# dps/rust-raytracer

Measured on NVIDIA H100. Metric: Mrays/sec (primary+scattered), higher is better.
Workload: dtype f64

## Files before the change

rust-raytracer_b200/csrc/rtb200_trace.cuh:

```cuda
#pragma once
#include "rtb200_kernels.cuh"

namespace rtk {

using namespace rtd;

#ifndef RT_SCATTER_TRIPS
#define RT_SCATTER_TRIPS 2
#endif
#ifndef RT_SMEM_STACK
#define RT_SMEM_STACK 10
#endif

enum : uint32_t { CLS_MISS = 0, CLS_DIFFUSE = 1, CLS_METAL = 2, CLS_GLASS = 3, CLS_LIGHT = 4, CLS_DEAD = 5, N_CLS = 6 };
constexpr uint32_t kDeadLevel = 0xffffffffu;
constexpr uint32_t kScatterPending = 0x80000000u;
using rtbvh::kLeafBit;
constexpr unsigned long long kNoHitBits = 0x7ff0000000000000ull;
constexpr uint32_t kNoSphere = 0xffffffffu;
using rtbvh::kSkipNodeBit;
using rtbvh::kNoSkip;
constexpr uint32_t kSlotBytes = 7 * 8 + 10 * 4 + RT_SMEM_STACK * 4;
constexpr uint32_t kFrameSlotBytes = 4;

struct Pool {
    double *ox, *oy, *oz, *dx, *dy, *dz, *bt;
    uint32_t *bi, *work, *pix, *smp, *blk, *clo, *chi, *lvl, *shd;
    uint32_t *src;
    uint32_t *stk;
    uint32_t *frm;
    uint32_t n_slots;
    uint32_t stack_col;
};
RT_DEV Pool pool_at(unsigned char* base, uint32_t n_slots, uint32_t stack_col) {
    Pool P;
    double* d = reinterpret_cast<double*>(base);
    P.ox = d; P.oy = d + n_slots; P.oz = d + 2 * n_slots; P.dx = d + 3 * n_slots; P.dy = d + 4 * n_slots; P.dz = d + 5 * n_slots; P.bt = d + 6 * n_slots;
    uint32_t* u = reinterpret_cast<uint32_t*>(d + 7 * n_slots);
    P.bi = u; P.work = u + n_slots; P.pix = u + 2 * n_slots; P.smp = u + 3 * n_slots; P.blk = u + 4 * n_slots; P.clo = u + 5 * n_slots;
    P.chi = u + 6 * n_slots; P.lvl = u + 7 * n_slots; P.shd = u + 8 * n_slots; P.src = u + 9 * n_slots; P.stk = u + 10 * n_slots;
    P.frm = u + (10 + RT_SMEM_STACK) * n_slots;
    P.n_slots = n_slots; P.stack_col = stack_col;
    return P;
}

struct WarpCtx {
    float4 *cA, *cB, *cC;
    uint32_t *skip;
    uint32_t *l_in, *l_lf, *l_cd;
};
constexpr uint32_t kWarpCtxBytes = (3 * 32 * 16 + 32 * 4 + (uint32_t)(kCapIn + kCapLf + kCapCd) * 4 + 15u) & ~15u;
RT_DEV WarpCtx warpctx_at(unsigned char* base) {
    WarpCtx W;
    W.cA = reinterpret_cast<float4*>(base); W.cB = W.cA + 32; W.cC = W.cB + 32;
    W.skip = reinterpret_cast<uint32_t*>(W.cC + 32);
    W.l_in = W.skip + 32; W.l_lf = W.l_in + kCapIn; W.l_cd = W.l_lf + kCapLf;
    return W;
}

struct SceneRefs {
    const float4* nodes; const float4* leaf_rec; const uint32_t* leaf_id; const float4* filt;
    const double4* geo; const DevMat* mat;
};

struct Stats {
    uint32_t rays = 0, cand = 0, ovf = 0, samples = 0, leaves = 0, nodes = 0;
#if RT_PHASE_CLOCKS
    unsigned long long t_node = 0, t_leaf = 0, t_exact = 0;
    uint32_t exact_steps = 0, exact_tests = 0, src_skips = 0;
#endif
};

RT_DEV void bulk_stage(void* dst, const void* src, uint32_t bytes, uint64_t* bar) {
    const uint32_t CH = 32768u;
    for (uint32_t o = 0; o < bytes; o += CH) {
        uint32_t nb = bytes - o < CH ? bytes - o : CH;
        tma_bulk_g2s((char*)dst + o, (const char*)src + o, nb, bar);
    }
}

RT_DEV void albedo_of(uint32_t code, const DevMat* mat, float& r, float& g, float& b) {
    if (code == 0xffffffffu) { r = g = b = 1.0f; return; }
    if (code & 0x80000000u) {
        r = __fdiv_rn((float)(code & 0xffu), 255.0f);
        g = __fdiv_rn((float)((code >> 8) & 0xffu), 255.0f);
        b = __fdiv_rn((float)((code >> 16) & 0xffu), 255.0f);
    } else {
        const DevMat& m = mat[code];
        r = m.r; g = m.g; b = m.b;
    }
}

RT_DEV float fmax3(float a, float b, float c) { return fmaxf(fmaxf(a, b), c); }
RT_DEV float fmin3(float a, float b, float c) { return fminf(fminf(a, b), c); }

RT_DEV uint32_t warp_scan_incl(uint32_t v, int lane) {
#pragma unroll
    for (int off = 1; off < 32; off <<= 1) {
        uint32_t t = __shfl_up_sync(0xffffffffu, v, off);
        if (lane >= off) v += t;
    }
    return v;
}

RT_DEV float2 fma2_rn(float2 a, float2 b, float2 c) { return make_float2(__fmaf_rn(a.x, b.x, c.x), __fmaf_rn(a.y, b.y, c.y)); }

#define RT_FILTER_PAIRS(REC, DV, NP)                                                                                                  \
    _Pragma("unroll") for (int q = 0; q < (NP); ++q) {                                                                              \
        float4 A_ = (REC)[2 * q], B_ = (REC)[2 * q + 1];                                                                             \
        float2 cx = make_float2(A_.x, A_.y), cy = make_float2(A_.z, A_.w), cz = make_float2(B_.x, B_.y), nk = make_float2(B_.z, B_.w); \
        float2 bb = fma2_rn(cz, dz2, nod2);                                                                                          \
        float2 tt = fma2_rn(cz, oz2, nk);                                                                                            \
        bb = fma2_rn(cy, dy2, bb);                                                                                                   \
        tt = fma2_rn(cy, oy2, tt);                                                                                                   \
        bb = fma2_rn(cx, dx2, bb);                                                                                                   \
        tt = fma2_rn(cx, ox2, tt);                                                                                                   \
        (DV)[q] = fma2_rn(bb, bb, tt);                                                                                               \
    }

RT_DEV uint32_t class_of(uint32_t kind) {
    return (kind == RT_METAL) ? CLS_METAL : (kind == RT_GLASS) ? CLS_GLASS : (kind == RT_LIGHT) ? CLS_LIGHT : CLS_DIFFUSE;
}

template <uint32_t MODE, bool ANY = false>
RT_DEV uint32_t closest_hit(const TraceParams& p, const SceneRefs& sc, const Pool& P, const WarpCtx& W, bool alive, uint32_t slot, int lane, Stats& st,
                            double t_hi = DBL_MAX, float* tcap = nullptr) {
    const unsigned FULL = 0xffffffffu;
    uint32_t cls = CLS_DEAD;
    if (__ballot_sync(FULL, alive) == 0u) return cls;
    const uint32_t lt_mask = (1u << lane) - 1u;
    unsigned long long* btu = reinterpret_cast<unsigned long long*>(P.bt);
    const D3 o = mk(P.ox[slot], P.oy[slot], P.oz[slot]), d = mk(P.dx[slot], P.dy[slot], P.dz[slot]);
    const double a = length_squared(d);
    const double thi = ANY ? t_hi : DBL_MAX;
    bool ovf = false;
    uint32_t done = 0u;
    double best_t = DBL_MAX;
    int best = -1;
    auto confirm = [&](int j) {
        if constexpr (ANY) { if (best >= 0) return; }
        double4 gq = sc.geo[j];
        double root;
        if (sphere_root(mk(gq.x, gq.y, gq.z), gq.w, o, d, a, 0.001, thi, root)) {
            if (best < 0 || root < best_t || (root == best_t && j < best)) { best_t = root; best = j; }
        }
        ++st.cand;
    };
    if (alive) { btu[slot] = kNoHitBits; P.bi[slot] = 0xffffffffu; }
    if (MODE != MODE_EXACT) {
        const float ofx = __double2float_rn(__dsub_rn(o.x, p.gx)), ofy = __double2float_rn(__dsub_rn(o.y, p.gy)),
                    ofz = __double2float_rn(__dsub_rn(o.z, p.gz));
        const float dfx = __double2float_rn(d.x), dfy = __double2float_rn(d.y), dfz = __double2float_rn(d.z);
        const float s = fmaf(dfx, dfx, fmaf(dfy, dfy, dfz * dfz));
        const float oo = fmaf(ofx, ofx, fmaf(ofy, ofy, ofz * ofz));
        const bool ok = (s > 1e-30f) && (s < 1e30f) && (oo < 1e30f);
        const float inv = rsqrtf(s);
        const float dnx = dfx * inv, dny = dfy * inv, dnz = dfz * inv;
        const float nod = -fmaf(ofx, dnx, fmaf(ofy, dny, ofz * dnz));
        const float thr = __fmul_rd(oo, p.er_coef);
        if (alive && !ok) ovf = true;
        if (MODE == MODE_TREE) {
            const float ax = fabsf(dnx) < 1e-20f ? copysignf(1e-20f, dnx) : dnx;
            const float ay = fabsf(dny) < 1e-20f ? copysignf(1e-20f, dny) : dny;
            const float az = fabsf(dnz) < 1e-20f ? copysignf(1e-20f, dnz) : dnz;
            const float mray = __fmul_ru(1.9073486328125e-6f, __fsqrt_ru(oo));
            W.cA[lane] = make_float4(ofx, ofy, ofz, mray);
            W.cB[lane] = make_float4(__frcp_rn(ax), __frcp_rn(ay), __frcp_rn(az), thr);
            W.cC[lane] = make_float4(dnx, dny, dnz, nod);
            if constexpr (ANY) tcap[lane] = __double2float_ru(__dmul_ru(__dmul_ru(t_hi, __dsqrt_ru(a)), 1.0 + 0x1p-40));
            uint32_t skp = kNoSkip;
            const uint32_t src = alive ? P.src[slot] : kNoSphere;
            if (src != kNoSphere) {
                const uint32_t pos = p.skip_pos[src];
                const double4 gs = sc.geo[src];
                if (pos != kNoSkip && leaves_sphere(mk(gs.x, gs.y, gs.z), gs.w, o, d, a)) skp = pos;
            }
            W.skip[lane] = skp;
            const uint32_t fat_in = (uint32_t)kCapIn - 7u * p.depth - 8u;
            const bool enter = alive && ok && p.n_nodes != 0u;
            const unsigned em = __ballot_sync(FULL, enter);
            uint32_t n_in = (uint32_t)__popc(em), n_lf = 0u, n_cd = 0u;
            if (enter) W.l_in[__popc(em & lt_mask)] = (uint32_t)lane;
            __syncwarp();
            uint32_t guard = 0;
            for (;;) {
#if RT_PHASE_CLOCKS
                const unsigned long long t_step = clock64();
#endif
                if (n_in != 0u && n_lf <= (uint32_t)(kCapLf - 64)) {
                    const uint32_t m = n_in < 32u ? n_in : 32u;
                    const bool act = (uint32_t)lane < m;
                    const uint32_t e = act ? W.l_in[n_in - 1u - (uint32_t)lane] : 0u;
                    const uint32_t ray = e & 31u, node = e >> 5;
                    uint32_t hit = 0u, leafbits = 0u;
                    const float4* N = sc.nodes + (size_t)node * kNodeVec;
                    bool test = act;
                    if constexpr (ANY) test = act && !((done >> ray) & 1u);
                    if (test) {
                        const float4 A = W.cA[ray], B = W.cB[ray];
                        float tcr = 0.f;
                        if constexpr (ANY) tcr = tcap[ray];
                        auto far_ = [&](float f) { if constexpr (ANY) return fminf(f, tcr); else return f; };
                        const uint32_t sx = __float_as_uint(B.x) >> 31, sy = __float_as_uint(B.y) >> 31, sz = __float_as_uint(B.z) >> 31;
                        const float mx = copysignf(A.w, B.x), my = copysignf(A.w, B.y), mz = copysignf(A.w, B.z);
                        const float cnx = __fmul_rn(__fadd_rn(A.x, mx), -B.x), cfx = __fmul_rn(__fsub_rn(A.x, mx), -B.x);
                        const float cny = __fmul_rn(__fadd_rn(A.y, my), -B.y), cfy = __fmul_rn(__fsub_rn(A.y, my), -B.y);
                        const float cnz = __fmul_rn(__fadd_rn(A.z, mz), -B.z), cfz = __fmul_rn(__fsub_rn(A.z, mz), -B.z);
                        const float2 ix2 = make_float2(B.x, B.x), iy2 = make_float2(B.y, B.y), iz2 = make_float2(B.z, B.z);
                        const float2 cnx2 = make_float2(cnx, cnx), cny2 = make_float2(cny, cny), cnz2 = make_float2(cnz, cnz);
                        const float2 cfx2 = make_float2(cfx, cfx), cfy2 = make_float2(cfy, cfy), cfz2 = make_float2(cfz, cfz);
                        const float4* Nnx = N + (sx ? 6 : 0); const float4* Nfx = N + (sx ? 0 : 6);
                        const float4* Nny = N + (sy ? 8 : 2); const float4* Nfy = N + (sy ? 2 : 8);
                        const float4* Nnz = N + (sz ? 10 : 4); const float4* Nfz = N + (sz ? 4 : 10);
#pragma unroll
                        for (int h = 0; h < 2; ++h) {
                            const float4 NX = Nnx[h], NY = Nny[h], NZ = Nnz[h], FX = Nfx[h], FY = Nfy[h], FZ = Nfz[h];
                            const float2 tnx0 = fma2_rn(make_float2(NX.x, NX.y), ix2, cnx2), tnx1 = fma2_rn(make_float2(NX.z, NX.w), ix2, cnx2);
                            const float2 tny0 = fma2_rn(make_float2(NY.x, NY.y), iy2, cny2), tny1 = fma2_rn(make_float2(NY.z, NY.w), iy2, cny2);
                            const float2 tnz0 = fma2_rn(make_float2(NZ.x, NZ.y), iz2, cnz2), tnz1 = fma2_rn(make_float2(NZ.z, NZ.w), iz2, cnz2);
                            const float2 tfx0 = fma2_rn(make_float2(FX.x, FX.y), ix2, cfx2), tfx1 = fma2_rn(make_float2(FX.z, FX.w), ix2, cfx2);
                            const float2 tfy0 = fma2_rn(make_float2(FY.x, FY.y), iy2, cfy2), tfy1 = fma2_rn(make_float2(FY.z, FY.w), iy2, cfy2);
                            const float2 tfz0 = fma2_rn(make_float2(FZ.x, FZ.y), iz2, cfz2), tfz1 = fma2_rn(make_float2(FZ.z, FZ.w), iz2, cfz2);
                            hit |= (fmaxf(fmax3(tnx0.x, tny0.x, tnz0.x), 0.f) <= far_(fmin3(tfx0.x, tfy0.x, tfz0.x)) ? 1u : 0u) << (4 * h + 0);
                            hit |= (fmaxf(fmax3(tnx0.y, tny0.y, tnz0.y), 0.f) <= far_(fmin3(tfx0.y, tfy0.y, tfz0.y)) ? 1u : 0u) << (4 * h + 1);
                            hit |= (fmaxf(fmax3(tnx1.x, tny1.x, tnz1.x), 0.f) <= far_(fmin3(tfx1.x, tfy1.x, tfz1.x)) ? 1u : 0u) << (4 * h + 2);
                            hit |= (fmaxf(fmax3(tnx1.y, tny1.y, tnz1.y), 0.f) <= far_(fmin3(tfx1.y, tfy1.y, tfz1.y)) ? 1u : 0u) << (4 * h + 3);
                        }
                        const uint4 R0 = *reinterpret_cast<const uint4*>(N + kChildVec), R1 = *reinterpret_cast<const uint4*>(N + kChildVec + 1);
                        leafbits = (R0.x >> 31) | ((R0.y >> 31) << 1) | ((R0.z >> 31) << 2) | ((R0.w >> 31) << 3) |
                                   ((R1.x >> 31) << 4) | ((R1.y >> 31) << 5) | ((R1.z >> 31) << 6) | ((R1.w >> 31) << 7);
                    }
                    {
                        const uint32_t sk = W.skip[ray] ^ (kSkipNodeBit | node << 3);
                        if (sk < 8u) {
#if RT_PHASE_CLOCKS
                            st.src_skips += (hit >> sk) & 1u;
#endif
                            hit &= ~(1u << sk);
                        }
                    }
                    const uint32_t packed = (uint32_t)__popc(hit & ~leafbits) | ((uint32_t)__popc(hit & leafbits) << 16);
                    const uint32_t inc = warp_scan_incl(packed, lane);
                    const uint32_t new_in = n_in - ((uint32_t)lane + 1u) + (inc & 0xffffu);
                    const bool fits = new_in <= (lane == 0 ? (uint32_t)kCapIn : fat_in) && n_lf + (inc >> 16) <= (uint32_t)kCapLf;
                    const unsigned okm = __ballot_sync(FULL, fits || !act);
                    uint32_t k = okm == FULL ? 32u : (uint32_t)(__ffs(~okm) - 1);
                    k = k < m ? k : m;
                    if (k == 0u) { if (lane == 0) atomicAdd(&p.err[1], 1ull); break; }
                    const uint32_t tot = __shfl_sync(FULL, inc, (int)k - 1);
                    __syncwarp();
                    if (act && (uint32_t)lane < k) {
                        const uint32_t exc = inc - packed;
                        uint32_t pi = (n_in - k) + (exc & 0xffffu), pl = n_lf + (exc >> 16);
                        const uint32_t* refs = reinterpret_cast<const uint32_t*>(N + kChildVec);
                        uint32_t mm = hit;
                        while (mm) {
                            const int c = __ffs(mm) - 1;
                            mm &= mm - 1u;
                            const uint32_t ref = refs[c];
                            if (ref & kLeafBit) W.l_lf[pl++] = (ref << 5) | ray;
                            else W.l_in[pi++] = (ref << 5) | ray;
                        }
                        if constexpr (ANY) st.nodes += test ? 1u : 0u; else ++st.nodes;
                    }
                    n_in = n_in - k + (tot & 0xffffu);
                    n_lf += tot >> 16;
                    __syncwarp();
#if RT_PHASE_CLOCKS
                    if (lane == 0) st.t_node += clock64() - t_step;
#endif
                } else if (n_lf != 0u && n_cd <= (uint32_t)(kCapCd - 32)) {
                    const uint32_t m = n_lf < 32u ? n_lf : 32u;
                    const bool act = (uint32_t)lane < m;
                    const uint32_t e = act ? W.l_lf[n_lf - 1u - (uint32_t)lane] : 0u;
                    const uint32_t ray = e & 31u, leaf = e >> 5;
                    uint32_t hit = 0u;
                    bool test = act;
                    if constexpr (ANY) test = act && !((done >> ray) & 1u);
                    if (test) {
                        const float4 A = W.cA[ray], C = W.cC[ray];
                        const float th = W.cB[ray].w;
                        const float2 dx2 = make_float2(C.x, C.x), dy2 = make_float2(C.y, C.y), dz2 = make_float2(C.z, C.z);
                        const float2 ox2 = make_float2(2.f * A.x, 2.f * A.x), oy2 = make_float2(2.f * A.y, 2.f * A.y), oz2 = make_float2(2.f * A.z, 2.f * A.z);
                        const float2 nod2 = make_float2(C.w, C.w);
                        float2 Dv[kLeafK / 2];
                        const float4* rec = sc.leaf_rec + (size_t)leaf * kLeafK;
                        RT_FILTER_PAIRS(rec, Dv, kLeafK / 2)
#pragma unroll
                        for (int q = 0; q < kLeafK / 2; ++q) hit |= (Dv[q].x >= th ? 1u : 0u) << (2 * q) | (Dv[q].y >= th ? 1u : 0u) << (2 * q + 1);
                        const uint32_t sk = W.skip[ray];
                        if (sk / (uint32_t)kLeafK == leaf) {
#if RT_PHASE_CLOCKS
                            st.src_skips += (hit >> (sk % (uint32_t)kLeafK)) & 1u;
#endif
                            hit &= ~(1u << (sk % (uint32_t)kLeafK));
                        }
                    }
                    const uint32_t cntc = (uint32_t)__popc(hit);
                    const uint32_t inc = warp_scan_incl(cntc, lane);
                    const bool fits = n_cd + inc <= (uint32_t)kCapCd;
                    const unsigned okm = __ballot_sync(FULL, fits || !act);
                    uint32_t k = okm == FULL ? 32u : (uint32_t)(__ffs(~okm) - 1);
                    k = k < m ? k : m;
                    if (k == 0u) { if (lane == 0) atomicAdd(&p.err[1], 1ull); break; }
                    const uint32_t tot = __shfl_sync(FULL, inc, (int)k - 1);
                    if (act && (uint32_t)lane < k) {
                        uint32_t pc = n_cd + inc - cntc;
                        const uint32_t* ids = sc.leaf_id + (size_t)leaf * kLeafK;
                        uint32_t mm = hit;
                        while (mm) {
                            const int c = __ffs(mm) - 1;
                            mm &= mm - 1u;
                            W.l_cd[pc++] = (ids[c] << 5) | ray;
                        }
                        if constexpr (ANY) st.leaves += test ? 1u : 0u; else ++st.leaves;
                    }
                    n_lf -= k;
                    n_cd += tot;
                    __syncwarp();
#if RT_PHASE_CLOCKS
                    if (lane == 0) st.t_leaf += clock64() - t_step;
#endif
                } else if (n_cd != 0u) {
                    const uint32_t m = n_cd < 32u ? n_cd : 32u;
                    const bool act = (uint32_t)lane < m;
                    const uint32_t e = act ? W.l_cd[n_cd - 1u - (uint32_t)lane] : 0u;
                    const uint32_t rs = __shfl_sync(FULL, slot, (int)(e & 31u)), sph = e >> 5;
                    if constexpr (ANY) {
                        const uint32_t ray = e & 31u;
                        const double tr = __shfl_sync(FULL, t_hi, (int)ray);
                        bool acc = false;
                        if (act && !((done >> ray) & 1u)) {
                            const D3 ro = mk(P.ox[rs], P.oy[rs], P.oz[rs]), rd = mk(P.dx[rs], P.dy[rs], P.dz[rs]);
                            const double4 gq = sc.geo[sph];
                            double root;
                            acc = sphere_root(mk(gq.x, gq.y, gq.z), gq.w, ro, rd, length_squared(rd), 0.001, tr, root);
                            ++st.cand;
#if RT_PHASE_CLOCKS
                            ++st.exact_tests;
#endif
                        }
                        if (acc) P.bi[rs] = sph;
                        done |= __reduce_or_sync(FULL, acc ? 1u << ray : 0u);
                        n_cd -= m;
                        __syncwarp();
                        if ((em & ~done) == 0u) break;
                    } else {
                        unsigned long long key = ~0ull;
                        if (act) {
                            const D3 ro = mk(P.ox[rs], P.oy[rs], P.oz[rs]), rd = mk(P.dx[rs], P.dy[rs], P.dz[rs]);
                            const double4 gq = sc.geo[sph];
                            double root;
                            if (sphere_root(mk(gq.x, gq.y, gq.z), gq.w, ro, rd, length_squared(rd), 0.001, DBL_MAX, root)) key = (unsigned long long)__double_as_longlong(root);
                            ++st.cand;
#if RT_PHASE_CLOCKS
                            ++st.exact_tests;
#endif
                        }
                        const bool h = key != ~0ull;
                        const unsigned long long before = h ? btu[rs] : 0ull;
                        __syncwarp();
                        if (h && key < before) atomicMin(&btu[rs], key);
                        __syncwarp();
                        const bool mine = h && key == btu[rs];
                        if (mine && key < before) atomicMax(&P.bi[rs], 0xffffffffu);
                        __syncwarp();
                        if (mine) atomicMin(&P.bi[rs], sph);
                        n_cd -= m;
                        __syncwarp();
                    }
#if RT_PHASE_CLOCKS
                    if (lane == 0) { st.t_exact += clock64() - t_step; ++st.exact_steps; }
#endif
                } else {
                    break;
                }
                if (++guard > (1u << 22)) { if (lane == 0) atomicAdd(&p.err[1], 1ull); break; }
            }
        } else {
            if (alive && ok) {
                const float2 dx2 = make_float2(dnx, dnx), dy2 = make_float2(dny, dny), dz2 = make_float2(dnz, dnz);
                const float2 ox2 = make_float2(2.f * ofx, 2.f * ofx), oy2 = make_float2(2.f * ofy, 2.f * ofy), oz2 = make_float2(2.f * ofz, 2.f * ofz);
                const float2 nod2 = make_float2(nod, nod);
#pragma unroll 1
                for (uint32_t pp = 0; pp < p.n_pairs; pp += 4) {
                    float2 Dv[4];
                    const float4* rec = sc.filt + 2 * pp;
                    RT_FILTER_PAIRS(rec, Dv, 4)
#pragma unroll
                    for (int q = 0; q < 4; ++q) {
                        const uint32_t j = 2u * (pp + (uint32_t)q);
                        if (Dv[q].x >= thr && j < p.n) confirm((int)j);
                        if (Dv[q].y >= thr && j + 1u < p.n) confirm((int)j + 1);
                    }
                    if constexpr (ANY) { if (best >= 0) break; }
                }
            }
        }
    } else {
        ovf = alive;
    }
    if (alive) {
        if constexpr (ANY) { if ((done >> lane) & 1u) best = (int)P.bi[slot]; }
        if (ovf) {
            ++st.ovf;
            for (int k = 0; k < (int)p.n; ++k) {
                confirm(k);
                if constexpr (ANY) { if (best >= 0) break; }
            }
        } else if (MODE == MODE_TREE) {
            for (uint32_t k = 0; k < p.n_always; ++k) {
                if constexpr (ANY) { if (best >= 0) break; }
                confirm((int)p.always[k]);
            }
        }
        if constexpr (ANY) {
            if (best >= 0) P.bi[slot] = (uint32_t)best;
            ++st.rays;
            return CLS_MISS;
        }
        const unsigned long long tb = btu[slot];
        const uint32_t ti = P.bi[slot];
        if (best >= 0) {
            const unsigned long long kb = (unsigned long long)__double_as_longlong(best_t);
            if (ti == 0xffffffffu || kb < tb || (kb == tb && (uint32_t)best < ti)) { P.bt[slot] = best_t; P.bi[slot] = (uint32_t)best; }
        }
        const uint32_t fin = P.bi[slot];
        cls = CLS_MISS;
        if (fin != 0xffffffffu) cls = class_of(sc.mat[fin].kind);
        ++st.rays;
    }
    return cls;
}

template <bool LENS = false>
RT_DEV void primary_ray(const TraceParams& p, const rt_camera& cam, const rt_lens& lens, uint32_t k0, uint32_t k1, uint32_t x,
                        uint32_t y_local, uint32_t s0, uint32_t s_local, Rng& rng, D3& o, D3& d) {
    const uint32_t band_rows = p.band_rows, width = p.width, height = p.height;
    uint32_t band = y_local / band_rows;
    uint32_t y = (band * (uint32_t)p.world + (uint32_t)p.rank) * band_rows + (y_local - band * band_rows);
    rng_init(rng, y * width + x, s0 + s_local);
    double xi1 = rng_f64(rng, k0, k1);
    double u = __ddiv_rn(__dadd_rn((double)x, xi1), __dsub_rn((double)width, 1.0));
    double xi2 = rng_f64(rng, k0, k1);
    double v = __ddiv_rn(__dsub_rn((double)height, __dadd_rn((double)y, xi2)), __dsub_rn((double)height, 1.0));
    get_ray(cam, u, v, o, d);
    if constexpr (LENS) {
        if (lens.radius != 0.0) lens_apply(lens, rng.pixel, rng.sample, k0, k1, o, d);
    }
}

template <bool LIGHTS, uint32_t QUEUE, bool LENS = false>
RT_DEV bool regenerate_slot(const TraceParams& p, const Pool& P, bool want, uint32_t s, int lane, bool& exhausted, Stats& st,
                            uint32_t n_list = 0u) {
    constexpr bool FRAMES = QUEUE == Q_FRAMES;
    const unsigned FULL = 0xffffffffu;
    want = want && !exhausted;
    unsigned need = __ballot_sync(FULL, want);
    if (!need) return false;
    int leader = __ffs(need) - 1;
    unsigned base = 0;
    if (lane == leader) base = atomicAdd(p.work_counter, (unsigned)__popc(need));
    base = __shfl_sync(FULL, base, leader);
    if (base + (unsigned)__popc(need) >= (QUEUE == Q_LIST ? n_list * p.s_count : p.total_work)) exhausted = true;
    if (!want) return false;
    unsigned my = base + __popc(need & ((1u << lane) - 1u));
    if (my >= (QUEUE == Q_LIST ? n_list * p.s_count : p.total_work)) return false;
    uint32_t f = 0u, k0 = p.key0, k1 = p.key1;
    uint32_t x, s_local, y_local, lp, k_list = 0u;
    Rng rng;
    D3 o, d;
    if constexpr (QUEUE == Q_RAYS) {
        const uint32_t i = my % p.npix_local;
        rng_init(rng, p.stream0 + i, p.s0 + my / p.npix_local);
        rng.blk = 1u;
        const double* ro = p.ray_o + 3 * (size_t)i;
        const double* rd = p.ray_d + 3 * (size_t)i;
        o = mk(ro[0], ro[1], ro[2]);
        d = mk(rd[0], rd[1], rd[2]);
    } else {
        if constexpr (FRAMES) { f = my / p.frame_work; my -= f * p.frame_work; k0 = p.ftab[f].key0; k1 = p.ftab[f].key1; }
        if constexpr (QUEUE == Q_LIST) {
            s_local = my % p.s_count;
            k_list = n_list - 1u - my / p.s_count;
            lp = p.list[k_list];
            y_local = lp / p.width;
            x = lp - y_local * p.width;
        } else {
            x = my % p.width;
            const uint32_t t_ = my / p.width;
            s_local = t_ % p.s_count;
            const uint32_t rr = t_ / p.s_count;
            y_local = p.rows_local - 1u - rr;
            lp = y_local * p.width + x;
        }
        if constexpr (FRAMES) primary_ray<LENS>(p, p.ftab[f].cam, LENS ? p.ltab[f] : p.lens, k0, k1, x, y_local, p.s0, s_local, rng, o, d);
        else primary_ray<LENS>(p, p.cam, p.lens, k0, k1, x, y_local, p.s0, s_local, rng, o, d);
    }
    P.ox[s] = o.x; P.oy[s] = o.y; P.oz[s] = o.z; P.dx[s] = d.x; P.dy[s] = d.y; P.dz[s] = d.z;
    if constexpr (FRAMES) { P.work[s] = (f * p.s_count + s_local) * p.npix_local + lp; P.frm[s] = f; }
    else if constexpr (QUEUE == Q_LIST) P.work[s] = s_local * n_list + k_list;
    else if constexpr (QUEUE == Q_RAYS) P.work[s] = my;
    else P.work[s] = s_local * p.npix_local + lp;
    P.pix[s] = rng.pixel; P.smp[s] = rng.sample;
    P.blk[s] = (rng.blk << 1) | rng.has; P.clo[s] = rng.c_lo; P.chi[s] = rng.c_hi;
    P.lvl[s] = 0u;
    P.shd[s] = 0u;
    P.src[s] = kNoSphere;
    if (LIGHTS) {
        for (int q = 0; q < 6; ++q) p.lterm[(size_t)q * p.stack_stride + P.stack_col + s] = 0.0f;
    }
    ++st.samples;
    return true;
}

template <bool LIGHTS, bool FRAMES>
RT_DEV bool shade_slot(const TraceParams& p, const SceneRefs& sc, const Pool& P, uint32_t s, uint32_t c) {
    uint32_t k0 = p.key0, k1 = p.key1;
    if constexpr (FRAMES) { const FrameRec& fr = p.ftab[P.frm[s]]; k0 = fr.key0; k1 = fr.key1; }
    const DevMat* mat = sc.mat;
    const double4* geo = sc.geo;
    const size_t col = (size_t)P.stack_col + s;
    auto stack_push = [&](uint32_t lvl, uint32_t code) {
        if (lvl < (uint32_t)RT_SMEM_STACK) P.stk[lvl * P.n_slots + s] = code; else p.stack[(size_t)lvl * p.stack_stride + col] = code;
    };
    auto stack_get = [&](uint32_t lvl) -> uint32_t {
        return lvl < (uint32_t)RT_SMEM_STACK ? P.stk[lvl * P.n_slots + s] : p.stack[(size_t)lvl * p.stack_stride + col];
    };
    Rng rng; rng.pixel = P.pix[s]; rng.sample = P.smp[s];
    { uint32_t bh = P.blk[s]; rng.blk = bh >> 1; rng.has = bh & 1u; }
    rng.c_lo = P.clo[s]; rng.c_hi = P.chi[s];
    bool done = false;
    D3 o = mk(P.ox[s], P.oy[s], P.oz[s]), d = mk(P.dx[s], P.dy[s], P.dz[s]);
    uint32_t level = P.lvl[s];
    uint32_t shd = LIGHTS ? (P.shd[s] & ~kScatterPending) : 0u;
    const uint32_t rays_sample = level + 1u;
    float cr = 0.f, cg = 0.f, cb = 0.f;
    bool have_tc = false;
    float tr = 0.f, tg = 0.f, tb = 0.f;
    bool state_dirty = false;
    if (c == CLS_MISS) {
        float x, y, z;
        sky_color(d, length(d), p.sky_mode, p.sky, x, y, z);
        if (shd == 0u) { cr = x; cg = y; cb = z; done = true; }
        else { tr = x; tg = y; tb = z; have_tc = true; }
    } else {
        const uint32_t best = P.bi[s];
        const double best_t = P.bt[s];
        double4 gq = geo[best];
        const D3 center = mk(gq.x, gq.y, gq.z);
        HitRec h = hit_record(center, gq.w, o, d, best_t);
        const DevMat m = mat[best];
        uint32_t code = best;
        D3 nd = d;
        bool absorbed = false;
        const bool is_light = (c == CLS_LIGHT);
        D3 rs = mk(0, 0, 0);
        if (c == CLS_DIFFUSE || c == CLS_METAL) {
            const unsigned group = __activemask();
            const bool sampled = random_in_unit_sphere_ilp<RT_SCATTER_TRIPS>(rng, k0, k1, rs);
            __syncwarp(group);
            if (!sampled) {
                P.blk[s] = (rng.blk << 1) | rng.has; P.clo[s] = rng.c_lo; P.chi[s] = rng.c_hi;
                P.shd[s] |= kScatterPending;
                return false;
            }
        }
        if (c == CLS_DIFFUSE) {
            D3 sd = add(h.normal, rs);
            if (near_zero(sd)) sd = h.normal;
            D3 target = add(h.point, sd);
            nd = sub(target, h.point);
            if (m.kind == RT_TEXTURE) {
                double tu, tv;
                sphere_uv(sub(h.point, center), tu, tv);
                code = 0x80000000u | texture_texel(p.tex[m.tex], m.param, tu, tv);
            }
        } else if (c == CLS_METAL) {
            D3 refl = reflect(d, h.normal);
            nd = add(refl, mul(rs, m.param));
            if (!(dot(nd, h.normal) > 0.0)) absorbed = true;
        } else if (c == CLS_GLASS) {
            double ratio = h.front_face ? __ddiv_rn(1.0, m.param) : m.param;
            D3 ud = unit_vector(d);
            double cos_theta = fmin(dot(neg(ud), h.normal), 1.0);
            double sin_theta = __dsqrt_rn(__dsub_rn(1.0, __dmul_rn(cos_theta, cos_theta)));
            bool refl = __dmul_rn(ratio, sin_theta) > 1.0;
            if (!refl) refl = reflectance(cos_theta, ratio) > rng_f64(rng, k0, k1);
            nd = refl ? reflect(ud, h.normal) : refract(ud, h.normal, ratio);
        }
        state_dirty = true;
        if (absorbed) {
            if (shd == 0u) done = true;
            else have_tc = true;
        } else {
            bool pass = false;
            if (LIGHTS) {
                const double prob = (c == CLS_GLASS) ? 0.05 : 0.1;
                const double xi = rng_f64(rng, k0, k1);
                const unsigned long long depth_now = (unsigned long long)p.max_depth - level;
                const bool depth_ok = (shd > 0u) ? true : (depth_now > (unsigned long long)p.max_depth - 2ull);
                pass = (xi > __dsub_rn(1.0, __dmul_rn((double)p.n_lights, prob))) && depth_ok;
                if (pass && shd >= p.max_shadow) { pass = false; atomicAdd(&p.err[0], 1ull); }
            }
            if (pass) {
                float ar, ag, ab;
                albedo_of(is_light ? 0xffffffffu : code, mat, ar, ag, ab);
                ShadowFrame f;
                f.px = h.point.x; f.py = h.point.y; f.pz = h.point.z; f.ndx = nd.x; f.ndy = nd.y; f.ndz = nd.z;
                f.ar = ar; f.ag = ag; f.ab = ab; f.sr = 0.f; f.sg = 0.f; f.sb = 0.f; f.li = 0u; f.code = code; f.is_light = is_light ? 1u : 0u; f.pad = 0u;
                p.frames[(size_t)shd * p.stack_stride + col] = f;
                ++shd;
                double4 lq = geo[p.lights[0]];
                o = h.point; d = sub(mk(lq.x, lq.y, lq.z), h.point);
                P.src[s] = best;
            } else if (shd == 0u) {
                if (is_light) { cr = 1.f; cg = 1.f; cb = 1.f; done = true; }
                else {
                    stack_push(level, code);
                    ++level;
                    o = h.point; d = nd; P.src[s] = best;
                    if (level == p.max_depth) done = true;
                }
            } else {
                tr = tg = tb = is_light ? 1.f : 0.f;
                if (p.albedo_nonfinite && !is_light) {
                    float ar, ag, ab;
                    albedo_of(code, mat, ar, ag, ab);
                    tr = clampf(__fadd_rn(0.f, __fmul_rn(ar, 0.f))); tg = clampf(__fadd_rn(0.f, __fmul_rn(ag, 0.f))); tb = clampf(__fadd_rn(0.f, __fmul_rn(ab, 0.f)));
                }
                have_tc = true;
            }
        }
    }
    if (LIGHTS) {
        while (have_tc) {
            ShadowFrame f = p.frames[(size_t)(shd - 1u) * p.stack_stride + col];
            f.sr = __fadd_rn(f.sr, __fmul_rn(f.ar, tr)); f.sg = __fadd_rn(f.sg, __fmul_rn(f.ag, tg)); f.sb = __fadd_rn(f.sb, __fmul_rn(f.ab, tb));
            ++f.li;
            state_dirty = true;
            if (f.li < p.n_lights) {
                p.frames[(size_t)(shd - 1u) * p.stack_stride + col] = f;
                double4 lq = geo[p.lights[f.li]];
                o = mk(f.px, f.py, f.pz); d = sub(mk(lq.x, lq.y, lq.z), o);
                P.src[s] = kNoSphere;
                have_tc = false;
            } else {
                const float nl = (float)p.n_lights;
                const float Lr = __fdiv_rn(f.sr, nl), Lg = __fdiv_rn(f.sg, nl), Lb = __fdiv_rn(f.sb, nl);
                --shd;
                if (shd == 0u) {
                    have_tc = false;
                    if (f.is_light) { cr = 1.f; cg = 1.f; cb = 1.f; done = true; }
                    else {
                        p.lterm[(size_t)(level * 3u + 0u) * p.stack_stride + col] = Lr;
                        p.lterm[(size_t)(level * 3u + 1u) * p.stack_stride + col] = Lg;
                        p.lterm[(size_t)(level * 3u + 2u) * p.stack_stride + col] = Lb;
                        stack_push(level, f.code);
                        ++level;
                        o = mk(f.px, f.py, f.pz); d = mk(f.ndx, f.ndy, f.ndz);
                        P.src[s] = kNoSphere;
                        if (level == p.max_depth) done = true;
                    }
                } else if (f.is_light) { tr = tg = tb = 1.f; }
                else {
                    tr = clampf(__fadd_rn(Lr, __fmul_rn(f.ar, 0.0f))); tg = clampf(__fadd_rn(Lg, __fmul_rn(f.ag, 0.0f))); tb = clampf(__fadd_rn(Lb, __fmul_rn(f.ab, 0.0f)));
                }
            }
        }
    }
    if (state_dirty && !done) {
        P.ox[s] = o.x; P.oy[s] = o.y; P.oz[s] = o.z; P.dx[s] = d.x; P.dy[s] = d.y; P.dz[s] = d.z;
        P.blk[s] = (rng.blk << 1) | rng.has; P.clo[s] = rng.c_lo; P.chi[s] = rng.c_hi;
        P.lvl[s] = level;
        P.shd[s] = shd;
    }
    if (done) {
        if (LIGHTS || p.albedo_nonfinite || cr != 0.f || cg != 0.f || cb != 0.f) {
            for (int l = (int)level - 1; l >= 0; --l) {
                float ar, ag, ab;
                albedo_of(stack_get((uint32_t)l), mat, ar, ag, ab);
                float Lr = 0.f, Lg = 0.f, Lb = 0.f;
                if (LIGHTS && l < 2) {
                    Lr = p.lterm[(size_t)(l * 3 + 0) * p.stack_stride + col];
                    Lg = p.lterm[(size_t)(l * 3 + 1) * p.stack_stride + col];
                    Lb = p.lterm[(size_t)(l * 3 + 2) * p.stack_stride + col];
                }
                cr = clampf(__fadd_rn(Lr, __fmul_rn(ar, cr)));
                cg = clampf(__fadd_rn(Lg, __fmul_rn(ag, cg)));
                cb = clampf(__fadd_rn(Lb, __fmul_rn(ab, cb)));
            }
        }
        p.samplebuf[P.work[s]] = make_float4(cr, cg, cb, __uint_as_float(rays_sample));
        P.lvl[s] = kDeadLevel;
    }
    return done;
}

RT_DEV void flush_stats(const TraceParams& p, const Stats& st, int lane) {
    unsigned long long v[6] = {st.rays, st.cand, st.ovf, st.samples, st.leaves, st.nodes};
#pragma unroll
    for (int k = 0; k < 6; ++k) {
#pragma unroll
        for (int off = 16; off > 0; off >>= 1) v[k] += __shfl_down_sync(0xffffffffu, v[k], off);
    }
    if (lane == 0) {
        atomicAdd(&p.stat[0], v[0]);
        atomicAdd(&p.stat[1], v[1]);
        atomicAdd(&p.stat[2], v[2]);
        atomicAdd(&p.stat[3], v[3]);
        atomicAdd(&p.stat[4], v[4]);
        atomicAdd(&p.stat[6], v[5]);
    }
#if RT_PHASE_CLOCKS
    unsigned long long w[6] = {st.t_node, st.t_leaf, st.t_exact, st.exact_steps, st.exact_tests, st.src_skips};
#pragma unroll
    for (int k = 0; k < 6; ++k) {
#pragma unroll
        for (int off = 16; off > 0; off >>= 1) w[k] += __shfl_down_sync(0xffffffffu, w[k], off);
    }
    if (lane == 0) {
#pragma unroll
        for (int k = 0; k < 6; ++k) atomicAdd(&p.stat[kPhaseStat + PH_NODE + k], w[k]);
    }
#endif
}

}
```

rust-raytracer_b200/csrc/rtb200_wavefront.cu:

```cuda
#include <cstdio>
#include <cstdlib>

#include "rtb200_trace.cuh"

namespace rtk {

namespace {

struct WfSmem {
    uint32_t nodes_off, leafrec_off, leafid_off, filt_off, geo_off, mat_off;
    uint32_t warpctx;
    uint32_t pool;
    uint32_t perm;
    uint32_t cnt;
    uint32_t phase;
    uint32_t total;
};

template <uint32_t UNIT>
__host__ __device__ constexpr uint32_t stage_bytes(uint32_t count) { return UNIT % 16u == 0u ? count * UNIT : (count * UNIT + 15u) & ~15u; }

__host__ __device__ constexpr WfSmem wf_layout(uint32_t n, uint32_t n_pairs, uint32_t n_nodes, uint32_t n_leaves, uint32_t mode, uint32_t mask, bool frames) {
    WfSmem L{};
    uint32_t off = 16;
    L.nodes_off = off;   if (mode == MODE_TREE && (mask & 1u)) off += n_nodes * (uint32_t)(kNodeVec * 16);
    L.leafrec_off = off; if (mode == MODE_TREE && (mask & 1u)) off += n_leaves * (uint32_t)(kLeafK * 16);
    L.leafid_off = off;  if (mode == MODE_TREE && (mask & 1u)) off += stage_bytes<kLeafK * 4>(n_leaves);
    L.filt_off = off;    if (mode == MODE_BRUTE && (mask & 1u)) off += n_pairs * 32u;
    L.geo_off = off; if (mask & 2u) off += n * 32u;
    L.mat_off = off; if (mask & 4u) off += n * 32u;
    off = (off + 15u) & ~15u;
    L.warpctx = off; if (mode == MODE_TREE) off += (uint32_t)(kBlock / 32) * kWarpCtxBytes;
    L.pool = off; off += (kSlotBytes + (frames ? kFrameSlotBytes : 0u)) * (uint32_t)kBlock;
    L.perm = off; off += 5u * kBlock * 2u;
    L.cnt = off; off += 2u * 8u * 4u;
    L.phase = off; if (RT_PHASE_CLOCKS) off += (uint32_t)(kBlock / 32) * kPhaseN * 8u;
    L.total = off;
    return L;
}

}

size_t wavefront_smem_bytes(const TraceParams& p, uint32_t mode, uint32_t smem_mask, uint32_t queue) {
    return wf_layout(p.n, p.n_pairs, p.n_nodes, p.n_leaves, mode, smem_mask, base_queue(queue) == Q_FRAMES).total;
}

constexpr int wf_min_blocks(uint32_t mode) {
    const int n = (mode == MODE_TREE ? 3 : 2) * 256 / kBlock;
    return n > 0 ? n : 1;
}

constexpr uint32_t smem_alloc(uint32_t bytes) { return (bytes + 127u) / 128u * 128u + 1024u; }
static_assert(RT_PHASE_CLOCKS || 3u * smem_alloc(wf_layout(0, 0, 0, 0, MODE_TREE, 0u, false).total) <= 196u * 1024u,
              "three single-frame tree CTAs per SM must fit the 196 KiB carveout");

template <typename K>
static cudaError_t set_carveout(K kern, uint32_t mode, size_t smem) {
    static const char* forced = getenv("RTB200_WF_CARVEOUT");
    if (forced) return cudaFuncSetAttribute(kern, cudaFuncAttributePreferredSharedMemoryCarveout, atoi(forced));
    int dev = 0, max_sm = 0, reserved = 0;
    cudaError_t e = cudaGetDevice(&dev);
    if (e == cudaSuccess) e = cudaDeviceGetAttribute(&max_sm, cudaDevAttrMaxSharedMemoryPerMultiprocessor, dev);
    if (e == cudaSuccess) e = cudaDeviceGetAttribute(&reserved, cudaDevAttrReservedSharedMemoryPerBlock, dev);
    if (e != cudaSuccess) return e;
    const size_t need = (size_t)wf_min_blocks(mode) * ((smem + 127u) / 128u * 128u + (size_t)reserved);
    const int pct = need >= (size_t)max_sm ? 100 : (int)(need * 100u / (size_t)max_sm);
    e = cudaFuncSetAttribute(kern, cudaFuncAttributePreferredSharedMemoryCarveout, pct);
    if (e != cudaSuccess || pct == 100) return e;
    int nb = 0;
    e = cudaOccupancyMaxActiveBlocksPerMultiprocessor(&nb, kern, kBlock, smem);
    if (e != cudaSuccess || nb >= wf_min_blocks(mode)) return e;
    return cudaFuncSetAttribute(kern, cudaFuncAttributePreferredSharedMemoryCarveout, pct + 1);
}

template <uint32_t MODE, bool LIGHTS, uint32_t QUEUE_>
__global__ void __launch_bounds__(kBlock, wf_min_blocks(MODE)) rt_wavefront_kernel(const __grid_constant__ TraceParams p) {
    constexpr uint32_t QUEUE = base_queue(QUEUE_);
    constexpr bool LENS = QUEUE != QUEUE_;
    constexpr bool FRAMES = QUEUE == Q_FRAMES;
    extern __shared__ __align__(128) unsigned char smem_raw[];
    const WfSmem L = wf_layout(p.n, p.n_pairs, p.n_nodes, p.n_leaves, MODE, p.scene_in_smem, FRAMES);
    uint64_t* bar = reinterpret_cast<uint64_t*>(smem_raw);
    const bool tree_smem = (p.scene_in_smem & 1u) != 0u;
    SceneRefs sc;
    sc.nodes = (MODE == MODE_TREE && tree_smem) ? reinterpret_cast<const float4*>(smem_raw + L.nodes_off) : p.nodes;
    sc.leaf_rec = (MODE == MODE_TREE && tree_smem) ? reinterpret_cast<const float4*>(smem_raw + L.leafrec_off) : p.leaf_rec;
    sc.leaf_id = (MODE == MODE_TREE && tree_smem) ? reinterpret_cast<const uint32_t*>(smem_raw + L.leafid_off) : p.leaf_id;
    sc.filt = (MODE == MODE_BRUTE && tree_smem) ? reinterpret_cast<const float4*>(smem_raw + L.filt_off) : p.filt;
    sc.geo = (p.scene_in_smem & 2u) ? reinterpret_cast<const double4*>(smem_raw + L.geo_off) : p.geo;
    sc.mat = (p.scene_in_smem & 4u) ? reinterpret_cast<const DevMat*>(smem_raw + L.mat_off) : p.mat;
    const int tid = threadIdx.x;
    const int lane = tid & 31;
    const unsigned FULL = 0xffffffffu;
    const Pool P = pool_at(smem_raw + L.pool, (uint32_t)kBlock, blockIdx.x * (uint32_t)kBlock);
    const WarpCtx W = warpctx_at(smem_raw + L.warpctx + (uint32_t)(tid >> 5) * kWarpCtxBytes);
    uint16_t* s_perm = reinterpret_cast<uint16_t*>(smem_raw + L.perm);
    uint32_t* s_cnt = reinterpret_cast<uint32_t*>(smem_raw + L.cnt);

    if (tid == 0) mbar_init(bar, 1);
    if (tid < 16) s_cnt[tid] = 0;
    P.lvl[tid] = kDeadLevel;
    __syncthreads();
    if (tid == 0) {
        const uint32_t b_nodes = (MODE == MODE_TREE && tree_smem) ? p.n_nodes * (uint32_t)(kNodeVec * 16) : 0u;
        const uint32_t b_lrec = (MODE == MODE_TREE && tree_smem) ? p.n_leaves * (uint32_t)(kLeafK * 16) : 0u;
        const uint32_t b_lid = (MODE == MODE_TREE && tree_smem) ? stage_bytes<kLeafK * 4>(p.n_leaves) : 0u;
        const uint32_t b_filt = (MODE == MODE_BRUTE && tree_smem) ? p.n_pairs * 32u : 0u;
        const uint32_t b_geo = (p.scene_in_smem & 2u) ? p.n * 32u : 0u, b_mat = (p.scene_in_smem & 4u) ? p.n * 32u : 0u;
        mbar_arrive_expect_tx(bar, b_nodes + b_lrec + b_lid + b_filt + b_geo + b_mat);
        if (b_nodes) bulk_stage(smem_raw + L.nodes_off, p.nodes, b_nodes, bar);
        if (b_lrec) bulk_stage(smem_raw + L.leafrec_off, p.leaf_rec, b_lrec, bar);
        if (b_lid) bulk_stage(smem_raw + L.leafid_off, p.leaf_id, b_lid, bar);
        if (b_filt) bulk_stage(smem_raw + L.filt_off, p.filt, b_filt, bar);
        if (b_geo) bulk_stage(smem_raw + L.geo_off, p.geo, b_geo, bar);
        if (b_mat) bulk_stage(smem_raw + L.mat_off, p.mat, b_mat, bar);
    }
    mbar_wait(bar, 0);

    auto now_ns = []() { unsigned long long t; asm volatile("mov.u64 %0, %%globaltimer;" : "=l"(t)); return t; };
    if (tid == 0) atomicMin(&p.stat[8], now_ns());
    Stats st;
    bool exhausted = false;
    bool stamped = false;
    uint32_t dry_iters = 0;
    uint32_t n_list = 0u;
    if constexpr (QUEUE == Q_LIST) n_list = *p.list_n;
    regenerate_slot<LIGHTS, QUEUE, LENS>(p, P, true, (uint32_t)tid, lane, exhausted, st, n_list);
    __syncthreads();

#if RT_PHASE_CLOCKS
    static_assert(kPhaseStat + kPhaseN <= 32, "the per-launch stat block holds 32 counters");
    unsigned long long* ph = reinterpret_cast<unsigned long long*>(smem_raw + L.phase) + (uint32_t)(tid >> 5) * kPhaseN;
    if (lane < (int)kPhaseN) ph[lane] = 0ull;
    unsigned long long t_mark = clock64();
    auto tick = [&](uint32_t k) { __syncwarp(); const unsigned long long t = clock64(); if (lane == 0) ph[k] += t - t_mark; t_mark = t; };
#endif
    const uint32_t lt_mask = (1u << lane) - 1u;
    uint32_t it = 0;
    for (;; ++it) {
        uint32_t* cnt = s_cnt + (it & 1u) * 8u;
        const bool alive = P.lvl[tid] != kDeadLevel;
        const bool pending = alive && (P.shd[tid] & kScatterPending) != 0u;
        uint32_t cls = closest_hit<MODE>(p, sc, P, W, alive && !pending, (uint32_t)tid, lane, st);
        if (pending) cls = class_of(sc.mat[P.bi[tid]].kind);
#if RT_PHASE_CLOCKS
        tick(PH_HIT);
#endif

#pragma unroll
        for (uint32_t c = 0; c < CLS_DEAD; ++c) {
            unsigned b = __ballot_sync(FULL, cls == c);
            if (b) {
                uint32_t base = 0;
                if (lane == 0) base = atomicAdd(&cnt[c], (uint32_t)__popc(b));
                base = __shfl_sync(FULL, base, 0);
                if (cls == c) s_perm[c * (uint32_t)kBlock + base + (uint32_t)__popc(b & lt_mask)] = (uint16_t)tid;
            }
        }
        __syncthreads();
#if RT_PHASE_CLOCKS
        tick(PH_SORT_WAIT_A);
#endif
        uint32_t c0 = cnt[0], c1 = cnt[1], c2 = cnt[2], c3 = cnt[3], c4 = cnt[4];
        const uint32_t e0 = c0, e1 = e0 + c1, e2 = e1 + c2, e3 = e2 + c3, n_live = e3 + c4;
        if (tid < 8) s_cnt[((it + 1u) & 1u) * 8u + tid] = 0u;

        const bool active = (uint32_t)tid < n_live;
        const uint32_t c = !active ? CLS_DEAD : ((uint32_t)tid < e0 ? CLS_MISS : (uint32_t)tid < e1 ? CLS_DIFFUSE : (uint32_t)tid < e2 ? CLS_METAL : (uint32_t)tid < e3 ? CLS_GLASS : CLS_LIGHT);
        const uint32_t cstart = c == CLS_MISS ? 0u : c == CLS_DIFFUSE ? e0 : c == CLS_METAL ? e1 : c == CLS_GLASS ? e2 : e3;
        const uint32_t s = active ? (uint32_t)s_perm[c * (uint32_t)kBlock + ((uint32_t)tid - cstart)] : 0u;
        bool done = false;
        if (active) done = shade_slot<LIGHTS, FRAMES>(p, sc, P, s, c);
#if RT_PHASE_CLOCKS
        tick(PH_SHADE);
        {
            const bool scatter = active && (c == CLS_DIFFUSE || c == CLS_METAL);
            const unsigned sm = __ballot_sync(FULL, scatter), dm = __ballot_sync(FULL, scatter && !done && (P.shd[s] & kScatterPending) != 0u);
            if (lane == 0) { ph[PH_ITERS] += 1ull; ph[PH_SCATTERS] += (unsigned)__popc(sm); ph[PH_DEFERRED] += (unsigned)__popc(dm); }
        }
#endif
        regenerate_slot<LIGHTS, QUEUE, LENS>(p, P, active && done, s, lane, exhausted, st, n_list);
        if (exhausted && !stamped) { stamped = true; if (lane == 0) atomicMin(&p.stat[9], now_ns()); }
        if (stamped) ++dry_iters;
        const bool still_alive = active && (P.lvl[s] != kDeadLevel);
#if RT_PHASE_CLOCKS
        tick(PH_REGEN);
#endif
        const int more = __syncthreads_or(still_alive ? 1 : 0);
#if RT_PHASE_CLOCKS
        tick(PH_WAIT_C);
#endif
        if (!more) break;
    }
    flush_stats(p, st, lane);
#if RT_PHASE_CLOCKS
    __syncwarp();
    if (lane < (int)kPhaseN) atomicAdd(&p.stat[kPhaseStat + lane], ph[lane]);
#endif
    if (tid == 0) { atomicMax(&p.stat[10], now_ns()); atomicMax(&p.stat[11], (unsigned long long)dry_iters); atomicAdd(&p.stat[12], (unsigned long long)dry_iters); }
}

template <uint32_t QUEUE, typename F>
static auto dispatch_mode(uint32_t mode, bool lights, F&& f) {
    if (mode == MODE_EXACT) return lights ? f(rt_wavefront_kernel<MODE_EXACT, true, QUEUE>) : f(rt_wavefront_kernel<MODE_EXACT, false, QUEUE>);
    if (mode == MODE_BRUTE) return lights ? f(rt_wavefront_kernel<MODE_BRUTE, true, QUEUE>) : f(rt_wavefront_kernel<MODE_BRUTE, false, QUEUE>);
    return lights ? f(rt_wavefront_kernel<MODE_TREE, true, QUEUE>) : f(rt_wavefront_kernel<MODE_TREE, false, QUEUE>);
}
template <typename F>
static auto dispatch(uint32_t mode, bool lights, uint32_t queue, F&& f) {
    if (queue == Q_RAYS) return dispatch_mode<Q_RAYS>(mode, lights, f);
    if (queue == Q_LIST) return dispatch_mode<Q_LIST>(mode, lights, f);
    if (queue == Q_FRAMES_LENS) return dispatch_mode<Q_FRAMES_LENS>(mode, lights, f);
    if (queue == Q_LIST_LENS) return dispatch_mode<Q_LIST_LENS>(mode, lights, f);
    return queue == Q_FRAMES ? dispatch_mode<Q_FRAMES>(mode, lights, f) : dispatch_mode<Q_SINGLE>(mode, lights, f);
}

cudaError_t launch_wavefront(const TraceParams& p, uint32_t mode, uint32_t queue, int grid, size_t smem, cudaStream_t st) {
    return dispatch(mode, p.n_lights > 0, queue, [&](auto kern) -> cudaError_t {
        cudaError_t e = cudaFuncSetAttribute(kern, cudaFuncAttributeMaxDynamicSharedMemorySize, (int)smem);
        if (e == cudaSuccess) e = set_carveout(kern, mode, smem);
        if (e != cudaSuccess) return e;
        kern<<<grid, kBlock, smem, st>>>(p);
        return cudaGetLastError();
    });
}

int wavefront_max_ctas_per_sm(uint32_t mode, bool lights, uint32_t queue, size_t smem) {
    return dispatch(mode, lights, queue, [&](auto kern) -> int {
        int nb = 0;
        if (cudaFuncSetAttribute(kern, cudaFuncAttributeMaxDynamicSharedMemorySize, (int)smem) != cudaSuccess) { cudaGetLastError(); return 0; }
        if (set_carveout(kern, mode, smem) != cudaSuccess) { cudaGetLastError(); return 0; }
        if (cudaOccupancyMaxActiveBlocksPerMultiprocessor(&nb, kern, kBlock, smem) != cudaSuccess) { cudaGetLastError(); return 0; }
        return nb;
    });
}

cudaError_t wavefront_info(uint32_t mode, bool lights, uint32_t queue, KernelInfo* out) {
    return dispatch(mode, lights, queue, [&](auto kern) -> cudaError_t {
        cudaFuncAttributes a;
        cudaError_t e = cudaFuncGetAttributes(&a, kern);
        if (e != cudaSuccess) return e;
        out->registers = a.numRegs; out->max_threads = a.maxThreadsPerBlock; out->const_bytes = (int)a.constSizeBytes; out->local_bytes = (int)a.localSizeBytes;
        const uint32_t bq = base_queue(queue);
        snprintf(out->name, sizeof out->name, "rt_wavefront_kernel<%s,%s%s%s>",
                 mode == MODE_TREE ? "MODE_TREE" : mode == MODE_BRUTE ? "MODE_BRUTE" : "MODE_EXACT", lights ? "LIGHTS" : "NO_LIGHTS",
                 bq == Q_FRAMES ? ",FRAMES" : bq == Q_LIST ? ",LIST" : bq == Q_RAYS ? ",RAYS" : "", bq != queue ? ",LENS" : "");
        return cudaSuccess;
    });
}

}
```

Before: 5617.

## Claim work in per-block shared-memory windows instead of per-warp global atomics

Adds a per-block work window in shared memory that thread 0 refills each iteration by claiming a chunk of work indices from the global counter, sized by remaining work over the grid. Warps then take new ray indices with a shared-memory atomic on the window and fall back to the global counter only when the window runs out. The goal is to cut contention on the single global work counter. In exchange it adds more complex index bookkeeping, moves the mbarrier and shrinks the counter arrays in the shared-memory layout, and may unbalance load near the end of the work.

Result: no change. 5594, median of 6 (-0.4%).

```diff
diff --git a/rust-raytracer_b200/csrc/rtb200_trace.cuh b/rust-raytracer_b200/csrc/rtb200_trace.cuh
--- a/rust-raytracer_b200/csrc/rtb200_trace.cuh
+++ b/rust-raytracer_b200/csrc/rtb200_trace.cuh
@@ -450,22 +450,59 @@
     }
 }
 
+struct WorkWindow {
+    uint32_t used, a0, a1, nn;
+};
+constexpr uint32_t kWindowChunk = 4u * (uint32_t)kBlock;
+constexpr uint32_t kWindowDry = 0x80000000u;
+static_assert(kWindowChunk + (uint32_t)kBlock < 0x8000u, "n0 and n1 fit their 15 bits");
+
+RT_DEV void window_refill(const TraceParams& p, WorkWindow* w, uint32_t n_work) {
+    const uint32_t nn = w->nn, n0 = nn & 0xffffu, n1 = (nn >> 16) & 0x7fffu, u = min(w->used, n0 + n1);
+    uint32_t a0 = w->a0 + u, r0 = n0 - u, a1 = w->a1, r1 = n1, dry = nn & kWindowDry;
+    if (u >= n0) { a0 = a1 + (u - n0); r0 = n1 - (u - n0); r1 = 0u; }
+    if (!dry && r1 == 0u && r0 < (uint32_t)kBlock) {
+        const uint32_t c = *reinterpret_cast<volatile const uint32_t*>(p.work_counter);
+        uint32_t g = n_work;
+        uint32_t claim = 0u;
+        if (c < n_work) {
+            claim = min(kWindowChunk, max(32u, (n_work - c) / (2u * gridDim.x)));
+            g = atomicAdd(p.work_counter, claim);
+        }
+        if (g < n_work) { a1 = g; r1 = min(claim, n_work - g); }
+        if (g >= n_work || g + claim >= n_work) dry = kWindowDry;
+    }
+    w->a0 = a0; w->a1 = a1; w->nn = r0 | r1 << 16 | dry; w->used = 0u;
+}
+
 template <bool LIGHTS, uint32_t QUEUE, bool LENS = false>
-RT_DEV bool regenerate_slot(const TraceParams& p, const Pool& P, bool want, uint32_t s, int lane, bool& exhausted, Stats& st,
-                            uint32_t n_list = 0u) {
+RT_DEV bool regenerate_slot(const TraceParams& p, const Pool& P, WorkWindow* win, bool want, uint32_t s, int lane, bool& exhausted,
+                            Stats& st, uint32_t n_work, uint32_t n_list = 0u) {
     constexpr bool FRAMES = QUEUE == Q_FRAMES;
     const unsigned FULL = 0xffffffffu;
     want = want && !exhausted;
     unsigned need = __ballot_sync(FULL, want);
     if (!need) return false;
-    int leader = __ffs(need) - 1;
+    const int leader = __ffs(need) - 1;
+    const unsigned cnt = (unsigned)__popc(need);
     unsigned base = 0;
-    if (lane == leader) base = atomicAdd(p.work_counter, (unsigned)__popc(need));
+    if (lane == leader) base = atomicAdd(&win->used, cnt);
     base = __shfl_sync(FULL, base, leader);
-    if (base + (unsigned)__popc(need) >= (QUEUE == Q_LIST ? n_list * p.s_count : p.total_work)) exhausted = true;
+    const uint32_t nn = win->nn, n0 = nn & 0xffffu, avail = n0 + ((nn >> 16) & 0x7fffu);
+    const uint32_t past = max(base, avail);
+    unsigned g = n_work;
+    if (base + cnt >= avail) {
+        if (nn & kWindowDry) exhausted = true;
+        else if (base + cnt > avail) {
+            if (lane == leader) g = atomicAdd(p.work_counter, base + cnt - past);
+            g = __shfl_sync(FULL, g, leader);
+            if (g + (base + cnt - past) >= n_work) exhausted = true;
+        }
+    }
     if (!want) return false;
-    unsigned my = base + __popc(need & ((1u << lane) - 1u));
-    if (my >= (QUEUE == Q_LIST ? n_list * p.s_count : p.total_work)) return false;
+    const uint32_t i = base + __popc(need & ((1u << lane) - 1u));
+    unsigned my = i < n0 ? win->a0 + i : i < avail ? win->a1 + (i - n0) : g + (i - past);
+    if (my >= n_work) return false;
     uint32_t f = 0u, k0 = p.key0, k1 = p.key1;
     uint32_t x, s_local, y_local, lp, k_list = 0u;
     Rng rng;
diff --git a/rust-raytracer_b200/csrc/rtb200_wavefront.cu b/rust-raytracer_b200/csrc/rtb200_wavefront.cu
--- a/rust-raytracer_b200/csrc/rtb200_wavefront.cu
+++ b/rust-raytracer_b200/csrc/rtb200_wavefront.cu
@@ -80,7 +80,7 @@
     constexpr bool FRAMES = QUEUE == Q_FRAMES;
     extern __shared__ __align__(128) unsigned char smem_raw[];
     const WfSmem L = wf_layout(p.n, p.n_pairs, p.n_nodes, p.n_leaves, MODE, p.scene_in_smem, FRAMES);
-    uint64_t* bar = reinterpret_cast<uint64_t*>(smem_raw);
+    uint64_t* bar = reinterpret_cast<uint64_t*>(smem_raw + L.cnt + 2u * 5u * 4u);
     const bool tree_smem = (p.scene_in_smem & 1u) != 0u;
     SceneRefs sc;
     sc.nodes = (MODE == MODE_TREE && tree_smem) ? reinterpret_cast<const float4*>(smem_raw + L.nodes_off) : p.nodes;
@@ -96,10 +96,16 @@
     const WarpCtx W = warpctx_at(smem_raw + L.warpctx + (uint32_t)(tid >> 5) * kWarpCtxBytes);
     uint16_t* s_perm = reinterpret_cast<uint16_t*>(smem_raw + L.perm);
     uint32_t* s_cnt = reinterpret_cast<uint32_t*>(smem_raw + L.cnt);
+    static_assert(sizeof(WorkWindow) <= 16u, "the work window fits the layout's first 16 B");
+    WorkWindow* win = reinterpret_cast<WorkWindow*>(smem_raw);
+    uint32_t n_list = 0u;
+    if constexpr (QUEUE == Q_LIST) n_list = *p.list_n;
+    const uint32_t n_work = QUEUE == Q_LIST ? n_list * p.s_count : p.total_work;
 
     if (tid == 0) mbar_init(bar, 1);
-    if (tid < 16) s_cnt[tid] = 0;
+    if (tid < 10) s_cnt[tid] = 0;
     P.lvl[tid] = kDeadLevel;
+    if (tid == 0) { *win = WorkWindow{}; window_refill(p, win, n_work); }
     __syncthreads();
     if (tid == 0) {
         const uint32_t b_nodes = (MODE == MODE_TREE && tree_smem) ? p.n_nodes * (uint32_t)(kNodeVec * 16) : 0u;
@@ -123,9 +129,7 @@
     bool exhausted = false;
     bool stamped = false;
     uint32_t dry_iters = 0;
-    uint32_t n_list = 0u;
-    if constexpr (QUEUE == Q_LIST) n_list = *p.list_n;
-    regenerate_slot<LIGHTS, QUEUE, LENS>(p, P, true, (uint32_t)tid, lane, exhausted, st, n_list);
+    regenerate_slot<LIGHTS, QUEUE, LENS>(p, P, win, true, (uint32_t)tid, lane, exhausted, st, n_work, n_list);
     __syncthreads();
 
 #if RT_PHASE_CLOCKS
@@ -138,7 +142,8 @@
     const uint32_t lt_mask = (1u << lane) - 1u;
     uint32_t it = 0;
     for (;; ++it) {
-        uint32_t* cnt = s_cnt + (it & 1u) * 8u;
+        uint32_t* cnt = s_cnt + (it & 1u) * 5u;
+        if (tid == 0) window_refill(p, win, n_work);
         const bool alive = P.lvl[tid] != kDeadLevel;
         const bool pending = alive && (P.shd[tid] & kScatterPending) != 0u;
         uint32_t cls = closest_hit<MODE>(p, sc, P, W, alive && !pending, (uint32_t)tid, lane, st);
@@ -163,7 +168,7 @@
 #endif
         uint32_t c0 = cnt[0], c1 = cnt[1], c2 = cnt[2], c3 = cnt[3], c4 = cnt[4];
         const uint32_t e0 = c0, e1 = e0 + c1, e2 = e1 + c2, e3 = e2 + c3, n_live = e3 + c4;
-        if (tid < 8) s_cnt[((it + 1u) & 1u) * 8u + tid] = 0u;
+        if (tid < 5) s_cnt[((it + 1u) & 1u) * 5u + tid] = 0u;
 
         const bool active = (uint32_t)tid < n_live;
         const uint32_t c = !active ? CLS_DEAD : ((uint32_t)tid < e0 ? CLS_MISS : (uint32_t)tid < e1 ? CLS_DIFFUSE : (uint32_t)tid < e2 ? CLS_METAL : (uint32_t)tid < e3 ? CLS_GLASS : CLS_LIGHT);
@@ -179,7 +184,7 @@
             if (lane == 0) { ph[PH_ITERS] += 1ull; ph[PH_SCATTERS] += (unsigned)__popc(sm); ph[PH_DEFERRED] += (unsigned)__popc(dm); }
         }
 #endif
-        regenerate_slot<LIGHTS, QUEUE, LENS>(p, P, active && done, s, lane, exhausted, st, n_list);
+        regenerate_slot<LIGHTS, QUEUE, LENS>(p, P, win, active && done, s, lane, exhausted, st, n_work, n_list);
         if (exhausted && !stamped) { stamped = true; if (lane == 0) atomicMin(&p.stat[9], now_ns()); }
         if (stamped) ++dry_iters;
         const bool still_alive = active && (P.lvl[s] != kDeadLevel);
```
